# seanwood/gcc-nmf

Hardware: AMD Instinct MI355X
Metric: stereo frames/sec (1024-FFT, K=1024, 100 NMF iters) (higher is better)
Workload: dtype f32; 1 GPU; HBM-resident (float32 samples in HBM -> separated float32 waveforms in HBM; the host-to-host rates are the host_to_host_* fields of a --full run): 64 x 10 s stereo @16 kHz synthetic mixtures per GPU (SURVEY 8d recipe), 1024-pt FFT hop 256 (F=513, T=622/file), K=1024, 100 KL-NMF iters, 128 TDOAs, 3 targets, independent dictionary per file; dictionary_size=1024, parallelism=file-sharded x1, no data-path collective

## Files before the change

### gcc_nmf_amd/csrc/common.h

```cpp
#pragma once
#include <hip/hip_runtime.h>
#include <stdint.h>

#define GCCNMF_OK 0
#define GCCNMF_ERR_ARG 1
#define GCCNMF_ERR_LAUNCH 2
#define GCCNMF_ERR_UNSUPPORTED 3

static inline int gccnmf_ceil_div(int a, int b) { return (a + b - 1) / b; }
static inline int gccnmf_round_up(int a, int b) { return gccnmf_ceil_div(a, b) * b; }

#define GCCNMF_CHECK_LAUNCH()                                   \
    do {                                                        \
        hipError_t e__ = hipGetLastError();                     \
        if (e__ != hipSuccess) return GCCNMF_ERR_LAUNCH;        \
    } while (0)

struct GccNmfPitches {
    int Fp, Kp, Np, Tp;
};

static inline GccNmfPitches gccnmf_make_pitches(int F, int T, int K) {
    GccNmfPitches p;
    p.Fp = gccnmf_round_up(F, 16);
    p.Kp = gccnmf_round_up(K, 64);
    p.Np = gccnmf_round_up(2 * T, 64);
    p.Tp = gccnmf_round_up(T, 64);
    return p;
}

#define GCCNMF_TUNE_KEYS 26
struct GccNmfTune {
    int v[GCCNMF_TUNE_KEYS];
};
extern thread_local GccNmfTune gccnmf_tune;
struct GccNmfCall {
    GccNmfCall();
    ~GccNmfCall();
};
#define GCCNMF_ENTER() GccNmfCall gccnmf_call_scope_
#define gccnmf_tune_ablate (gccnmf_tune.v[1])
#define gccnmf_tune_tile_policy (gccnmf_tune.v[2])
#define gccnmf_tune_dma (gccnmf_tune.v[3])
#define gccnmf_tune_ring (gccnmf_tune.v[4])
#define gccnmf_tune_wh_splits (gccnmf_tune.v[5])
#define gccnmf_tune_rht_splits (gccnmf_tune.v[6])
#define gccnmf_tune_exact_div (gccnmf_tune.v[7])
#define gccnmf_tune_shared_groups (gccnmf_tune.v[8])
#define gccnmf_tune_tail_split (gccnmf_tune.v[9])
#define gccnmf_tune_direct (gccnmf_tune.v[10])
#define gccnmf_tune_direct_tile (gccnmf_tune.v[11])
#define gccnmf_tune_direct_batch (gccnmf_tune.v[12])
#define gccnmf_tune_direct_depth (gccnmf_tune.v[13])
#define gccnmf_tune_short_updh (gccnmf_tune.v[14])
#define gccnmf_tune_fft_r16 (gccnmf_tune.v[15])
#define gccnmf_tune_fused_k12 (gccnmf_tune.v[16])
#define gccnmf_tune_fused_k34 (gccnmf_tune.v[17])
#define gccnmf_tune_persistent (gccnmf_tune.v[18])
#define gccnmf_tune_prefetch (gccnmf_tune.v[19])
#define gccnmf_tune_wide_update_w (gccnmf_tune.v[20])
#define gccnmf_tune_chain (gccnmf_tune.v[21])
#define gccnmf_tune_chain_solo (gccnmf_tune.v[22])
#define gccnmf_tune_chain_rag (gccnmf_tune.v[23])
#define gccnmf_tune_chain_chunk (gccnmf_tune.v[24])
#define gccnmf_tune_chain_fault (gccnmf_tune.v[25])
```

### gcc_nmf_amd/csrc/gemm_dma.h

```cpp
#pragma once
#include <mutex>
#include <type_traits>
#include "gemm_mfma.h"
#include "chain_sync.h"

#ifndef GEMM_DMA_ABL
#define GEMM_DMA_ABL 0
#endif

typedef __attribute__((address_space(3))) void* gemm_lds_ptr;
typedef __attribute__((address_space(1))) const void* gemm_glb_ptr;

__device__ __forceinline__ void gemm_dma16(const float* wave_uniform_base, unsigned lane_byte_offset, unsigned lds_wave_byte_addr) {
    asm volatile("s_mov_b32 m0, %2\n\tglobal_load_lds_dwordx4 %0, %1"
                 :
                 : "v"(lane_byte_offset), "s"(wave_uniform_base), "s"(lds_wave_byte_addr)
                 : "memory");
}

__device__ __forceinline__ void gemm_dma16_masked(const float* wave_uniform_base, unsigned lane_byte_offset, unsigned lds_wave_byte_addr,
                                                  unsigned long long wave_uniform_mask) {
    unsigned long long saved;
    asm volatile("s_mov_b64 %0, exec\n\ts_mov_b64 exec, %4\n\ts_mov_b32 m0, %3\n\tglobal_load_lds_dwordx4 %1, %2\n\ts_mov_b64 exec, %0"
                 : "=&s"(saved)
// ... 86 lines not shown
            if constexpr (NT == 4) v[e][1] = gemm_lds_read2_b32<64, 96>(base + 4 * e * ROWS);
        }
    }
    __device__ __forceinline__ void tie() {
#pragma unroll
        for (int e = 0; e < 4; ++e)
#pragma unroll
            for (int h = 0; h < NT / 2; ++h) gemm_tie(v[e][h]);
    }
    __device__ __forceinline__ void clear() {
#pragma unroll
        for (int e = 0; e < 4; ++e)
#pragma unroll
            for (int h = 0; h < NT / 2; ++h) v[e][h] = gemm_f32x2{0.f, 0.f};
    }
    __device__ __forceinline__ float get(int m, int e) const { return v[e][m >> 1][m & 1]; }
    __device__ __forceinline__ void scale(const gemm_f32x4& s) {
#pragma unroll
        for (int e = 0; e < 4; ++e)
#pragma unroll
            for (int h = 0; h < NT / 2; ++h) v[e][h] *= s[e];
    }
};

__device__ __forceinline__ float gemm_div_fast(float v, float d) {
    const float r = __builtin_amdgcn_rcpf(d);
    const float q = v * r;
    return fmaf(fmaf(-d, q, v), r, q);
}

typedef int gemm_i32x4 __attribute__((ext_vector_type(4)));
__device__ float gemm_buffer_load(gemm_i32x4 rsrc, int voffset, int soffset, int aux) __asm("llvm.amdgcn.raw.buffer.load.f32");
__device__ gemm_f32x4 gemm_buffer_load4(gemm_i32x4 rsrc, int voffset, int soffset, int aux) __asm("llvm.amdgcn.raw.buffer.load.v4f32");
__device__ void gemm_buffer_store(float data, gemm_i32x4 rsrc, int voffset, int soffset, int aux) __asm("llvm.amdgcn.raw.buffer.store.f32");
__device__ __forceinline__ gemm_i32x4 gemm_buffer_rsrc(const void* wave_uniform_base, long bytes = 0x7fffffffL) {
    const unsigned long long a = (unsigned long long)wave_uniform_base;
    gemm_i32x4 r;
    r.x = __builtin_amdgcn_readfirstlane((int)(unsigned)a);
    r.y = __builtin_amdgcn_readfirstlane((int)(unsigned)(a >> 32) & 0xffff);
    r.z = __builtin_amdgcn_readfirstlane((int)(bytes < 0x7fffffffL ? bytes : 0x7fffffffL));
    r.w = 0x00020000;
    return r;
}

template <int EPI, int BM = 512>
struct GemmEpiloguePair {
// ... 236 lines not shown
        q = idx / wt;
        const int w = idx - q * wt;
        tm = w / p.wide_n;
        col0 = (w - tm * p.wide_n) * 64 + 32 * half;
    } else {
        const int r = t - (len + s), base_r = list * p.cr;
        const int lenr = min(max(p.batch * p.rag * p.tiles_m - base_r, 0), p.cr);
        if (r >= lenr) return false;
        const int idx = base_r + r;
        q = idx / p.tiles_m;
        tm = idx - q * p.tiles_m;
        col0 = (p.tiles_n - 1) * 64;
        nw = 1;
    }
    file = gemm_dma_list_file(p, q) + p.file0;
    return true;
}

template <int TM>
struct GemmDmaLds {
    static constexpr int SBUF = 128 * TM * 16 + 64 * 16 + 16 + 16;
};

template <bool A_KC, bool B_KC, int EPI, bool TAIL, int TM, bool NARROW>
__device__ __forceinline__ void gemm_dma_workgroup(const GemmArgs& p, float* const smem, float* const s_rowvec, unsigned* const s_arrivals_p,
                                                   int* const s_ticket, const int list, int t, const GemmSync& sync, const int sync_it = 0,
                                                   const bool trace_on = true) {
    static_assert(TM == 4 || TM == 2, "");
    static_assert(TM == 4 || EPI != EPI_UPDW, "the fused W update owns all rows of its atoms: full-height tiles only");
    static_assert(!NARROW || (EPI != EPI_UPDW && TM == 4), "narrow items: full-height tiles with an element-wise epilogue");
    constexpr int BK = 16, BM = 128 * TM, BN = 64, RW = 32 * TM;
    constexpr int NA = 2 * TM;
    constexpr int SA = BM * BK, SB = BN * BK;
    constexpr int SBUF = SA + SB + BK + BK;
    static_assert(SBUF == GemmDmaLds<TM>::SBUF, "");
    constexpr bool SCALE = !B_KC && (EPI == EPI_DIV || EPI == EPI_STORE);
    unsigned& s_arrivals = *s_arrivals_p;

    int tid = threadIdx.x, lane = tid & 63;
    const int wave = __builtin_amdgcn_readfirstlane(tid >> 6);
    const int wm = wave, wn = 0;
    int l31 = lane & 31, hh = lane >> 5;
#ifdef GCCNMF_EXPERIMENTS
    const bool persistent = p.tickets != nullptr;
#else
    constexpr bool persistent = false;
#endif
// ... 269 lines not shown
        if (TAIL) {
            tail_acc = fmaf(t4.x, tb4.x, tail_acc);
            tail_acc = fmaf(t4.y, tb4.y, tail_acc);
            tail_acc = fmaf(t4.z, tb4.z, tail_acc);
            tail_acc = fmaf(t4.w, tb4.w, tail_acc);
        }
        if (B_KC) rowsum_acc += (rs4.x + rs4.y) + (rs4.z + rs4.w);
        __builtin_amdgcn_sched_barrier(0);
        GEMM_PROBE(6);
        wait_group0();
#ifdef GEMM_DMA_PROBE
        __builtin_amdgcn_sched_barrier(0);
        const unsigned long long pt7 = __builtin_amdgcn_s_memtime();
        probe[0] += pt1 - pt0;
        probe[1] += pt2 - pt1;
        probe[2] += pt3 - pt2;
        probe[3] += pt4 - pt3;
        probe[4] += pt5 - pt4;
        probe[5] += pt6 - pt5;
        probe[6] += pt7 - pt6;
        __builtin_amdgcn_sched_barrier(0);
#endif
    };
    auto main_loop = [&](auto nw_c) {
        for (int kt = 0; kt < nkt; kt += 2) {
            step(std::integral_constant<int, 0>{}, nw_c, kt);
            if (kt + 1 < nkt) step(std::integral_constant<int, 1>{}, nw_c, kt + 1);
        }
    };

    if (SCALE) {
        if (!p.bscale && tid < 2 * BK) smem[(tid >> 4) * SBUF + SA + SB + BK + (tid & 15)] = 1.f;
    }
    bool have = take_item(t);
    if (have) set_offsets(lane);
    bool prefetched = false;
    int it = 0;
    long long* trace_row = nullptr;
    while (have) {
        const int vb = p.lists == 8 ? 8 * t + list : t;
        trace_row = (trace_on && p.trace && vb < p.trace_rows) ? p.trace + 8 * (long)vb : nullptr;
        if (trace_row && tid == 0) {
            trace_row[0] = trace_row[1] = __builtin_amdgcn_s_memrealtime();
            trace_row[4] = (long long)((__builtin_amdgcn_s_getreg((3 << 11) | 20) & 15u) << 16 | (__builtin_amdgcn_s_getreg((31 << 11) | 4) & 0xffffu));
            trace_row[7] = (long long)blockIdx.x << 16 | (long long)it;
        }
#ifdef GCCNMF_EXPERIMENTS
        set_lane_constants(gemm_opaque_tid());
        if (it > 0) set_offsets(lane);
        a0.clear(); a1.clear(); b0.clear(); b1.clear();
        sc0 = sc1 = t4 = tb4 = ts4 = rs4 = zero4;
        tbxy = tbzw = gemm_f32x2{0.f, 0.f};
#else
        set_lane_constants(tid);
#endif
        gemm_sync_wait(sync, file, col0, tid, sync_it, list, n_sync);
        if (trace_row && tid == 0) trace_row[1] = __builtin_amdgcn_s_memrealtime();
        if (!prefetched) {
#pragma unroll
            for (int i = 0; i < NPIECES; ++i) dma_piece(i, 0, 0);
        }
#pragma unroll
        for (int m = 0; m < TM; ++m)
#pragma unroll
            for (int n = 0; n < 2; ++n)
#pragma unroll
                for (int r = 0; r < 16; ++r) acc[m][n][r] = 0.f;
        tail_acc = 0.f;
        rowsum_acc = 0.f;
        if constexpr (EPI == EPI_STORE || EPI == EPI_UPDH) {
#pragma unroll
            for (int i = 0; i < BM / 256; ++i) {
                const int lr = tid + 256 * i, row = min(row0 + lr, p.M - 1);
                s_rowvec[lr] = p.ktailA ? p.ktailA[file * p.s_ktailA + row] : 0.f;
                if (EPI == EPI_UPDH) {
                    const float rd = 1.0f / (p.E2[file * p.sE2 + row] + p.alpha + p.eps);
                    s_rowvec[BM + lr] = p.E1 ? p.E1[file * p.sE1 + row] * rd : rd;
                }
            }
        }
        if (tid == 0) {
            s_arrivals = 0;
            if (persistent) s_ticket[it & 1] = p.wpl + (int)__hip_atomic_fetch_add(p.tickets + list, 1u, __ATOMIC_RELAXED, __HIP_MEMORY_SCOPE_AGENT);
        }
        asm volatile("s_waitcnt vmcnt(0)" ::: "memory");
        __syncthreads();
        read_group0(lds0);
        wait_group0();

        if constexpr (NARROW) {
            if (nw == 1) main_loop(std::integral_constant<int, 1>{});
            else main_loop(std::integral_constant<int, 2>{});
        } else {
            main_loop(std::integral_constant<int, 2>{});
        }
        __syncthreads();
        if (trace_row && tid == 0) trace_row[2] = __builtin_amdgcn_s_memrealtime();

        const int e_file = file, e_row0 = row0, e_col0 = col0, e_nw = nw, e_n = n_item;
        const bool e_active = wave_active, e_tail = do_tail, e_rowsum = do_rowsum;
        have = false;
        prefetched = false;
        if (persistent) {
            t = __builtin_amdgcn_readfirstlane(s_ticket[it & 1]);
            have = take_item(t);
            if (have && p.prefetch) {
                set_offsets(gemm_opaque_tid() & 63);
#pragma unroll
                for (int i = 0; i < NPIECES; ++i) dma_piece(i, 0, 0);
                prefetched = true;
            }
// ... 66 lines not shown
            __syncthreads();
            if (tid == 0) trace_row[3] = __builtin_amdgcn_s_memrealtime();
        }
        gemm_sync_signal(sync, e_file, e_col0, e_nw, tid);
        ++it;
        if (have) __syncthreads();
    }
#ifdef GEMM_DMA_PROBE
    if (p.trace && lane == 0 && (long)p.trace_grid + 4L * blockIdx.x + 4 <= p.trace_rows) {
#pragma unroll
        for (int i = 0; i < 7; ++i) p.trace[8 * ((long)p.trace_grid + blockIdx.x * 4 + wave) + i] = (long long)probe[i];
        p.trace[8 * ((long)p.trace_grid + blockIdx.x * 4 + wave) + 7] = it;
    }
#endif
    if (persistent && tid == 0) {
        const unsigned gone = __hip_atomic_fetch_add(p.tickets + 8, 1u, __ATOMIC_ACQ_REL, __HIP_MEMORY_SCOPE_AGENT);
        if (gone == gridDim.x - 1) {
#pragma unroll
            for (int i = 0; i < 9; ++i) __hip_atomic_store(p.tickets + i, 0u, __ATOMIC_RELAXED, __HIP_MEMORY_SCOPE_AGENT);
        }
    }
}

template <bool A_KC, bool B_KC, int EPI, bool TAIL, int TM, bool NARROW>
__global__ __launch_bounds__(256, 2) void gccnmf_gemm_dma_kernel(GemmArgs p) {
    __shared__ __attribute__((aligned(16))) float smem[2 * GemmDmaLds<TM>::SBUF];
    __shared__ __attribute__((aligned(16))) float s_rowvec[(EPI == EPI_STORE || EPI == EPI_UPDH) ? 2 * 128 * TM : 4];
    __shared__ unsigned s_arrivals;
    __shared__ int s_ticket[2];
    const int list = p.lists == 8 ? (int)(blockIdx.x & 7) : 0;
    const int t = p.lists == 8 ? (int)(blockIdx.x >> 3) : (int)blockIdx.x;
    GemmSync none = {};
    gemm_dma_workgroup<A_KC, B_KC, EPI, TAIL, TM, NARROW>(p, smem, s_rowvec, &s_arrivals, s_ticket, list, t, none);
}

struct GemmChain {
    int first[5];
    int it0, iterations;
    int trace_it;
    GemmSync sync[4];
};
template <bool TAIL, int STAGES, int TM1>
__global__ __launch_bounds__(256, 2) void gccnmf_gemm_chain_kernel(GemmArgs p0, GemmArgs p1, GemmArgs p2, GemmArgs p3, GemmChain ch) {
    static_assert(STAGES == 2 || STAGES == 4, "");
    __shared__ __attribute__((aligned(16))) float smem[2 * GemmDmaLds<4>::SBUF];
    __shared__ __attribute__((aligned(16))) float s_rowvec[2 * 512];
    __shared__ unsigned s_arrivals;
    __shared__ int s_ticket[2];
    const int list = (int)(blockIdx.x & 7);
    int pos = (int)(blockIdx.x >> 3), it = ch.it0;
    if (ch.iterations > 1) {
        const int q = pos / ch.first[4];
        it += q;
        pos -= q * ch.first[4];
    }
    const bool tr = it == ch.trace_it;
    if (pos < ch.first[1]) {
        gemm_dma_workgroup<true, false, EPI_DIV, TAIL, 4, true>(p0, smem, s_rowvec, &s_arrivals, s_ticket, list, pos, ch.sync[0], it, tr);
    } else if (pos < ch.first[2]) {
        gemm_dma_workgroup<false, false, EPI_UPDH, false, TM1, TM1 == 4>(p1, smem, s_rowvec, &s_arrivals, s_ticket, list, pos - ch.first[1], ch.sync[1], it, tr);
    } else if constexpr (STAGES == 4) {
        if (pos < ch.first[3]) {
            gemm_dma_workgroup<true, false, EPI_DIV, TAIL, 4, true>(p2, smem, s_rowvec, &s_arrivals, s_ticket, list, pos - ch.first[2], ch.sync[2], it, tr);
        } else {
            gemm_dma_workgroup<true, true, EPI_UPDW, TAIL, 4, false>(p3, smem, s_rowvec, &s_arrivals, s_ticket, list, pos - ch.first[3], ch.sync[3], it, tr);
        }
    }
}

#ifdef GCCNMF_EXPERIMENTS
unsigned* gccnmf_ticket_block(hipStream_t stream);
#endif

static int gemm_dma_plan(GemmArgs& a, bool narrow_capable, int TM, int whole_files = 0) {
    a.tiles_m = gccnmf_ceil_div(a.M, 128 * TM);
    a.tiles_n = gccnmf_ceil_div(a.N, 64);
    a.lists = (a.xcd_affine && a.batch >= 8) ? 8 : 1;
    const int policy = gccnmf_tune_tail_split;
    const bool narrow_ok = narrow_capable && TM == 4 && policy != 0;
    a.narrow_ok = narrow_ok ? 1 : 0;
    const long tiles = (long)a.batch * a.tiles_m * a.tiles_n;
    if (tiles > (1L << 28)) return -1;
    a.rag = (narrow_ok && a.tiles_n >= 2 && a.N - (a.tiles_n - 1) * 64 <= 32) ? 1 : 0;
    if (a.rag && policy == 1 && !a.concurrent) {
        const long slots = a.lists == 8 ? 64 : 512;
        const long plain = (tiles + a.lists - 1) / a.lists;
        const long with_rag = ((long)a.batch * a.tiles_m * (a.tiles_n - 1) + a.lists - 1) / a.lists + ((long)a.batch * a.tiles_m + a.lists - 1) / a.lists;
        if ((with_rag + slots - 1) / slots > (plain + slots - 1) / slots) a.rag = 0;
// ... 22 lines not shown
    constexpr bool NARROW = false;
#else
    constexpr bool NARROW = TM == 4 && (EPI == EPI_DIV || EPI == EPI_UPDH || EPI == EPI_STORE);
#endif
    const int classic_grid = gemm_dma_plan(a, NARROW, TM);
    if (classic_grid < 1) return GCCNMF_ERR_ARG;
    a.trace = gccnmf_trace_buf;
    a.trace_rows = gccnmf_trace_buf ? gccnmf_trace_blocks : 0;
    a.trace_grid = classic_grid;
    a.tickets = nullptr;
    a.prefetch = 0;
    a.wpl = 0;
    int grid = classic_grid;
#ifdef GCCNMF_EXPERIMENTS
    a.prefetch = gccnmf_tune_prefetch;
    if (gccnmf_tune_persistent && TM == 4 && classic_grid > 512) {
        a.tickets = gccnmf_ticket_block(stream);
        if (a.tickets) {
            grid = 512;
            a.wpl = 512 / a.lists;
        }
    }
#endif
    hipLaunchKernelGGL((gccnmf_gemm_dma_kernel<A_KC, B_KC, EPI, TAIL, TM, NARROW>), dim3(grid), dim3(256), 0, stream, a);
    GCCNMF_CHECK_LAUNCH();
    return GCCNMF_OK;
}

template <bool A_KC, bool B_KC, int EPI, bool TAIL>
static int gccnmf_launch_gemm_dma(GemmArgs a, hipStream_t stream) {
    if (!a.A || !a.B || !a.C || a.M < 1 || a.N < 1 || a.Kd < 1 || a.batch < 1) return GCCNMF_ERR_ARG;
    if ((a.lda & 3) || (a.ldb & 3)) return GCCNMF_ERR_ARG;
    a.ablate = gccnmf_tune_ablate;
    a.exact_div = gccnmf_tune_exact_div;
    if constexpr (EPI != EPI_UPDW) {
        if ((a.M <= 256 && gccnmf_tune_tail_split != 0) || gccnmf_tune_tail_split == 3) return gccnmf_launch_gemm_dma_tm<A_KC, B_KC, EPI, TAIL, 2>(a, stream);
        const long tpf = (long)gccnmf_ceil_div(a.M, 512) * gccnmf_ceil_div(a.N, 64);
        const long total = tpf * a.batch, rounds = total / 512;
        if (gccnmf_tune_tail_split == 1 && !gccnmf_trace_buf && !a.concurrent && a.M > 256) {
            auto full_cost = [](long tiles) { const long r = tiles % 512; return (tiles / 512) * 250 + (r == 0 ? 0 : r <= 256 ? 135 : 250); };
            auto half_cost = [](long halves) {
                const long r = halves % 768;
                return (halves / 768) * 190 + (r == 0 ? 0 : r <= 256 ? 85 : r <= 512 ? 135 : 190);
            };
            const long plain = full_cost(total), all_half = half_cost(2 * total);
            long split = 1L << 40;
            const int head = (int)(rounds * 512 / tpf);
// ... 17 lines not shown
```

### gcc_nmf_amd/csrc/gemm_mfma.h

```cpp
#pragma once
#include "common.h"

typedef float f32x16 __attribute__((ext_vector_type(16)));

#ifndef GEMM_VARIANT
#define GEMM_VARIANT 2
#endif
#if GEMM_VARIANT & 1
#define GEMM_PRIO(x) __builtin_amdgcn_s_setprio(x)
#else
#define GEMM_PRIO(x)
#endif
#if GEMM_VARIANT & 2
#define GEMM_PIN()
#else
#define GEMM_PIN() __builtin_amdgcn_sched_barrier(0)
#endif

extern long long* gccnmf_trace_buf;
extern int gccnmf_trace_blocks;

enum GemmEpilogue {
    EPI_STORE = 0,
    EPI_DIV = 1,
// ... 34 lines not shown
    const float* E0;
    long sE0;
    const float* E1;
    long sE1;
    const float* E2;
    long sE2;
    const float2* X;
    long sX;
    float alpha, eps;
    int T, Tp, Fp, ldv;
    long long* trace;
    int lists;
    int cw, cr;
    int split;
    int rag, wide_n;
    int whole_files;
    const int* ragged_n;
    const int* ragged_lists;
    int ragged_kd;
    int narrow_ok;
    int wpl, prefetch;
    unsigned* tickets;
    int trace_rows, trace_grid;
};

template <int EPI>
__device__ __forceinline__ bool gemm_col_valid(const GemmArgs& p, int col) {
    if (EPI == EPI_PHASE) {
        int ic = col / p.Tp;
        return col < p.N && (col - ic * p.Tp) < p.T;
    }
    return col < p.N;
}

template <int EPI>
__device__ __forceinline__ void gemm_epilogue(const GemmArgs& p, int file, int row, int col, float acc) {
    if (EPI == EPI_STORE) {
        p.C[file * p.sC + (long)row * p.ldc + col] = acc;
    } else if (EPI == EPI_DIV) {
        long idx = (long)row * p.ldc + col;
        p.C[file * p.sC + idx] = p.E0[file * p.sE0 + idx] / acc;
    } else if (EPI == EPI_UPDH) {
        long idx = file * p.sC + (long)row * p.ldc + col;
        float h = p.C[idx];
        if (p.E1) h *= p.E1[file * p.sE1 + row];
        float den = p.E2[file * p.sE2 + row] + p.alpha + p.eps;
// ... 543 lines not shown
```

### gcc_nmf_amd/csrc/nmf.hip

```cpp
#include <mutex>
#include "gemm_ring.h"
#include "direct.h"
#include "update_w.h"
#ifdef GCCNMF_EXPERIMENTS
int gccnmf_launch_gemm_stream(GemmArgs a, hipStream_t stream);
#endif
int gccnmf_klnmf_fixed_launch(const float* V, const float* W, float* H, float* workspace, int F, int N, int K, int batch, int iterations,
                              float alpha, float eps, bool ones, hipStream_t s);
bool gccnmf_klnmf_fixed_supported(int F, int K);
long gccnmf_klnmf_fixed_workspace_floats(int F, int K);
#include "../../include/gccnmf_hip.h"

#include <atomic>
#include <algorithm>
#include <vector>
#define GCCNMF_SHARED_STREAMS 4
#define GCCNMF_CHAIN_MAX_ITERATIONS gccnmf_tune_chain_chunk
#define GCCNMF_RAGGED_MAX_BATCH 248
#define GCCNMF_SPLITS 4
#define GCCNMF_DIRECT_MAX_BATCH 8
struct GccNmfKnob {
    int def, lo, hi, experiment;
};
static const GccNmfKnob gccnmf_knobs[GCCNMF_TUNE_KEYS] = {
// ... 3 lines not shown
    {1, 0, 1, 0},
    {1, 0, 1, 1},
    {3, 1, 4, 1},
    {4, 1, 4, 1},
    {1, 0, 1, 0},
    {3, 1, GCCNMF_SHARED_STREAMS, 0},
    {1, 0, 3, 0},
    {1, 0, 1, 0},
    {0, 0, 8, 1},
    {4, 1, GCCNMF_DIRECT_MAX_BATCH, 0},
    {0, 0, 4, 1},
    {1, 0, 1, 1},
    {1, 0, 1, 1},
    {1, 0, 2, 0},
    {1, 0, 2, 0},
    {0, 0, 1, 1},
    {1, 0, 1, 1},
    {1, 0, 1, 1},
    {1, 0, 8, 0},
    {0, 0, 1, 1},
    {1, 0, 3, 0},
    {2048, 1, 65536, 0},
    {0, 0, 1, 1},
};
static std::atomic<int> gccnmf_knob_value[GCCNMF_TUNE_KEYS];
static std::atomic<int> gccnmf_knobs_ready{0};
static void gccnmf_knobs_init() {
    static std::mutex mu;
    if (gccnmf_knobs_ready.load(std::memory_order_acquire)) return;
    std::lock_guard<std::mutex> lock(mu);
    if (gccnmf_knobs_ready.load(std::memory_order_relaxed)) return;
    for (int k = 0; k < GCCNMF_TUNE_KEYS; ++k) gccnmf_knob_value[k].store(gccnmf_knobs[k].def, std::memory_order_relaxed);
    gccnmf_knobs_ready.store(1, std::memory_order_release);
}
static GccNmfTune gccnmf_tune_load() {
    gccnmf_knobs_init();
    GccNmfTune t;
    for (int k = 0; k < GCCNMF_TUNE_KEYS; ++k) t.v[k] = gccnmf_knob_value[k].load(std::memory_order_relaxed);
    return t;
}
thread_local GccNmfTune gccnmf_tune = gccnmf_tune_load();
static thread_local int gccnmf_call_depth = 0;
GccNmfCall::GccNmfCall() {
    if (gccnmf_call_depth++ == 0) gccnmf_tune = gccnmf_tune_load();
}
GccNmfCall::~GccNmfCall() { --gccnmf_call_depth; }
// ... 291 lines not shown
struct NmfGeom {
    int F, N, K, Fp, Kp, Np;
    int ld;
    int Fm;
    bool tail;
    long sV, sW, sH, sU;
};

static NmfGeom make_geom(int F, int N, int K) {
    NmfGeom g;
    GccNmfPitches p = gccnmf_make_pitches(F, 1, K);
    g.F = F; g.N = N; g.K = K;
    g.Fp = p.Fp; g.Kp = p.Kp; g.Np = gccnmf_round_up(N, 64);
    g.ld = g.Np;
    g.tail = (F % 128) == 1 && F > 1;
    g.Fm = g.tail ? F - 1 : F;
    g.sV = (long)g.Fp * g.Np;
    g.sW = (long)g.Fp * g.Kp;
    g.sH = (long)g.Kp * g.Np;
    g.sU = (long)g.Fp * g.Kp;
    return g;
}

static int launch_wh_div(const NmfGeom& g, const float* V, const float* W, long sW, const float* H, const float* hscale,
                         long sScale, float* R, int batch, int xcd, hipStream_t s) {
    GemmArgs a = {};
    a.A = W; a.sA = sW; a.lda = g.Kp; a.a_clamp = g.Fp - 1;
    a.B = H; a.sB = g.sH; a.ldb = g.ld; a.b_clamp = g.Np - 4;
    a.M = g.Fm; a.N = g.N; a.Kd = g.K;
    a.batch = batch; a.xcd_affine = xcd & 1; a.concurrent = (xcd >> 1) & 1;
    a.bscale = hscale; a.s_bscale = sScale;
    a.tail_row = g.F - 1;
    a.C = R; a.sC = g.sV; a.ldc = g.ld;
    a.E0 = V; a.sE0 = g.sV;
    return dispatch_gemm<true, false, EPI_DIV>(a, g.tail, s);
}

static int launch_update_h(const NmfGeom& g, const float* W, long sW, const float* R, float* H, const float* hscale,
                           long sScale, const float* colsumW, long sVec, float alpha, float eps, int batch, int xcd,
                           hipStream_t s) {
    GemmArgs a = {};
    a.A = W; a.sA = sW; a.lda = g.Kp; a.a_clamp = g.Kp - 4;
    a.B = R; a.sB = g.sV; a.ldb = g.ld; a.b_clamp = g.Np - 4;
    a.M = g.K; a.N = g.N; a.Kd = g.F;
    if ((g.F % 16) == 1) {
        a.Kd = g.F - 1;
        a.ktailA = W + (long)(g.F - 1) * g.Kp; a.s_ktailA = sW;
        a.ktailB = R + (long)(g.F - 1) * g.ld; a.s_ktailB = g.sV;
    }
    a.batch = batch; a.xcd_affine = xcd & 1; a.concurrent = (xcd >> 1) & 1;
    a.C = H; a.sC = g.sH; a.ldc = g.ld;
    a.E1 = hscale; a.sE1 = sScale;
    a.E2 = colsumW; a.sE2 = sVec;
    a.alpha = alpha; a.eps = eps;
    return dispatch_gemm<false, false, EPI_UPDH>(a, false, s);
}

static int launch_rht(const NmfGeom& g, const float* R, const float* H, float* U, float* rowsumH, int batch, int xcd,
                      hipStream_t s) {
    GemmArgs a = {};
    a.A = R; a.sA = g.sV; a.lda = g.ld; a.a_clamp = g.Fp - 1;
    a.B = H; a.sB = g.sH; a.ldb = g.ld; a.b_clamp = g.Kp - 1;
    a.M = g.Fm; a.N = g.K; a.Kd = g.N;
    a.batch = batch; a.xcd_affine = xcd & 1; a.concurrent = (xcd >> 1) & 1;
    a.tail_row = g.F - 1;
    a.rowsumB = rowsumH; a.s_rowsumB = g.Kp;
    a.C = U; a.sC = g.sU; a.ldc = g.Kp;
    return dispatch_gemm<true, true, EPI_STORE>(a, g.tail, s);
}

static bool can_fuse_w_update(const NmfGeom& g, int batch) {
    if (g.Fm <= 128 || g.Fm > 512 || gccnmf_tune_tile_policy == 2) return false;
    return gccnmf_tune_tile_policy == 1 || (long)batch * gccnmf_ceil_div(g.K, 64) >= 256;
}

static int launch_rht_update_w(const NmfGeom& g, const float* R, const float* H, float* W, float* colsumW, float* hscale, int batch,
                               int xcd, hipStream_t s) {
    GemmArgs a = {};
    a.A = R; a.sA = g.sV; a.lda = g.ld; a.a_clamp = g.Fp - 1;
    a.B = H; a.sB = g.sH; a.ldb = g.ld; a.b_clamp = g.Kp - 1;
    a.M = g.Fm; a.N = g.K; a.Kd = g.N;
    a.batch = batch; a.xcd_affine = xcd & 1; a.concurrent = (xcd >> 1) & 1;
    a.tail_row = g.F - 1;
    a.C = W; a.sC = g.sW; a.ldc = g.Kp;
    a.out_colsum = colsumW; a.out_norm = hscale; a.s_out = g.Kp;
    if (gccnmf_tune_dma && (a.M & 127) == 0 && (a.N & 63) == 0)
        return g.tail ? gccnmf_launch_gemm_dma<true, true, EPI_UPDW, true>(a, s) : gccnmf_launch_gemm_dma<true, true, EPI_UPDW, false>(a, s);
    return g.tail ? gccnmf_launch_gemm<4, 1, true, true, EPI_UPDW, true>(a, s) : gccnmf_launch_gemm<4, 1, true, true, EPI_UPDW, false>(a, s);
}

#ifdef GCCNMF_EXPERIMENTS

__global__ __launch_bounds__(256) void nmf_div_partials_kernel(const float* __restrict__ V, const float* __restrict__ P, long sP,
                                                               int nsplit, int F, int N, int Np, float* __restrict__ R) {
    const int n4 = Np / 4;
    const long idx = (long)blockIdx.x * 256 + threadIdx.x;
    if (idx >= (long)F * n4) return;
    const int f = (int)(idx / n4), n = 4 * (int)(idx - (long)f * n4);
    if (n >= N) return;
    const long i = (long)f * Np + n;
    float4 d = *(const float4*)(P + i);
// ... 218 lines not shown
    return any_size || can_fuse_w_update(g, batch);
}
static bool chain_rule(int batch, int flags) {
    if (flags & 4) return false;
    const int longest = (batch + 7) / 8;
    return batch >= 24 && 100L * 8 * longest <= 108L * batch;
}

struct RaggedPlan {
    const int* n;
    int lists[8][GEMM_RAGGED_LMAX + 1];
    const int* d_n;
    const int* d_lists;
};

static int launch_klnmf_chain(int stages, const NmfGeom& g, const float* V, float* W, float* H, float* R, float* colsumW, float* hscale,
                              float alpha, float eps, int batch, int flags, unsigned* counters, int it0, int iterations, hipStream_t s,
                              const RaggedPlan* rg = nullptr) {
    GemmArgs a[4] = {};
    const int concurrent = (flags & 4) ? 1 : 0;
    for (int i = 0; i < 4; ++i) {
        a[i].batch = batch; a[i].xcd_affine = 1; a[i].concurrent = concurrent;
        a[i].ablate = gccnmf_tune_ablate; a[i].exact_div = gccnmf_tune_exact_div;
    }
    for (int i = 0; i < 3; i += 2) {
        a[i].A = W; a[i].sA = g.sW; a[i].lda = g.Kp; a[i].a_clamp = g.Fp - 1;
        a[i].B = H; a[i].sB = g.sH; a[i].ldb = g.ld; a[i].b_clamp = g.Np - 4;
        a[i].M = g.Fm; a[i].N = g.N; a[i].Kd = g.K;
        a[i].tail_row = g.F - 1;
        a[i].C = R; a[i].sC = g.sV; a[i].ldc = g.ld;
        a[i].E0 = V; a[i].sE0 = g.sV;
    }
    a[0].bscale = hscale; a[0].s_bscale = g.Kp;
    a[1].A = W; a[1].sA = g.sW; a[1].lda = g.Kp; a[1].a_clamp = g.Kp - 4;
    a[1].B = R; a[1].sB = g.sV; a[1].ldb = g.ld; a[1].b_clamp = g.Np - 4;
    a[1].M = g.K; a[1].N = g.N; a[1].Kd = g.F - 1;
    a[1].ktailA = W + (long)(g.F - 1) * g.Kp; a[1].s_ktailA = g.sW;
    a[1].ktailB = R + (long)(g.F - 1) * g.ld; a[1].s_ktailB = g.sV;
    a[1].C = H; a[1].sC = g.sH; a[1].ldc = g.ld;
    a[1].E1 = hscale; a[1].sE1 = g.Kp;
    a[1].E2 = colsumW; a[1].sE2 = g.Kp;
    a[1].alpha = alpha; a[1].eps = eps;
    a[3].A = R; a[3].sA = g.sV; a[3].lda = g.ld; a[3].a_clamp = g.Fp - 1;
    a[3].B = H; a[3].sB = g.sH; a[3].ldb = g.ld; a[3].b_clamp = g.Kp - 1;
    a[3].M = g.Fm; a[3].N = g.K; a[3].Kd = g.N;
    a[3].tail_row = g.F - 1;
// ... 48 lines not shown
        ch.sync[2].sig_cnt = c34; ch.sync[2].sig_stride = 1; ch.sync[2].sig_per_tile = 0;
        ch.sync[3].wait_cnt = c34; ch.sync[3].wait_stride = 1; ch.sync[3].wait_per_tile = 0;
        ch.sync[3].wait_need = (unsigned)(a[2].tiles_m * (rg ? 1 : a[2].tiles_n));
        ch.sync[3].wait_scale_tiles = rg ? 1 : 0;
        {
            ch.sync[3].sig_cnt = c41; ch.sync[3].sig_stride = 1; ch.sync[3].sig_per_tile = 0;
            ch.sync[0].wait_cnt = c41; ch.sync[0].wait_stride = 1; ch.sync[0].wait_per_tile = 0; ch.sync[0].wait_lag = 1;
            ch.sync[0].wait_need = (unsigned)(a[3].tiles_m * a[3].tiles_n);
        }
    }
    if (iterations > 1 && stages != 4) return GCCNMF_ERR_ARG;
    if (it0 == 0 && iterations == 1) ch.sync[0].wait_cnt = nullptr;
    ch.it0 = it0; ch.iterations = iterations;
    ch.trace_it = it0 + (iterations > 4 ? iterations - 3 : iterations - 1);
    if ((long)8 * ch.first[4] * iterations > (1L << 30)) return GCCNMF_ERR_ARG;
    for (int i = 0; i < stages; ++i) {
        a[i].trace = gccnmf_trace_buf ? gccnmf_trace_buf + 8L * 8 * ch.first[i] : nullptr;
        a[i].trace_rows = gccnmf_trace_buf ? gccnmf_trace_blocks - 8 * ch.first[i] : 0;
        if (a[i].trace_rows <= 0) a[i].trace = nullptr;
    }
    const int grid = 8 * ch.first[4] * iterations;
    const unsigned pad = gccnmf_tune_chain_solo ? 16384u : 0u;
    if (!g.tail) return GCCNMF_ERR_ARG;
    if (stages == 2 && tm1 == 4) hipLaunchKernelGGL((gccnmf_gemm_chain_kernel<true, 2, 4>), dim3(grid), dim3(256), pad, s, a[0], a[1], a[2], a[3], ch);
    else if (stages == 2) hipLaunchKernelGGL((gccnmf_gemm_chain_kernel<true, 2, 2>), dim3(grid), dim3(256), pad, s, a[0], a[1], a[2], a[3], ch);
    else if (tm1 == 4) hipLaunchKernelGGL((gccnmf_gemm_chain_kernel<true, 4, 4>), dim3(grid), dim3(256), pad, s, a[0], a[1], a[2], a[3], ch);
    else hipLaunchKernelGGL((gccnmf_gemm_chain_kernel<true, 4, 2>), dim3(grid), dim3(256), pad, s, a[0], a[1], a[2], a[3], ch);
    GCCNMF_CHECK_LAUNCH();
    return GCCNMF_OK;
}

static int short_chain_group(const NmfGeom& g, int batch, int flags) {
    const int want = gccnmf_tune_chain;
    if (!want || want == 2 || want == 4 || !gccnmf_tune_fused_k12 || !gccnmf_tune_fused_k34 || gccnmf_tune_tile_policy != 0) return 0;
    if (direct_path(g, batch) || (flags & 3) || batch < 8 || !g.tail || g.Fm < 64 || g.Fm > 512 || (g.Fm % 64) != 0 || g.K > 128) return 0;
    if ((g.Fm / 64) * 16 < 32 * gccnmf_ceil_div(g.K, 32) || g.F > 64 * 9 || !gccnmf_tune_ring || (long)batch * (g.Kp / 64) >= 256) return 0;
    if (want == 1 && !(chain_rule(batch, flags) && fused_wh_updh(g, batch, flags) && fused_whdiv_rht_files(g, batch, flags) == batch)) return 0;
    if (gccnmf_tune_ablate == 64) return 0;
    return ((long)batch * (g.Kp / 32) >= 256 && gccnmf_tune_wide_update_w) ? 32 : 16;
}

static int launch_short_chain(const NmfGeom& g, const float* V, float* W, float* H, float* U, float* colsumW, float* rowsumH, float* hscale,
                              float alpha, float eps, int batch, int group, unsigned* counters, int it0, int iterations, hipStream_t s) {
    ShortChainArgs c = {};
    c.a12.W = W; c.a12.sW = g.sW; c.a12.lda = g.Kp;
    c.a12.H = H; c.a12.sH = g.sH; c.a12.ldb = g.ld;
    c.a12.V = V; c.a12.sV = g.sV; c.a12.ldv = g.ld;
    c.a12.scale = hscale; c.a12.colsum = colsumW; c.a12.sVec = g.Kp;
    c.a12.M = g.Fm; c.a12.N = g.N; c.a12.Kd = g.K; c.a12.batch = batch;
    c.a12.alpha = alpha; c.a12.eps = eps;
// ... 674 lines not shown
```

Measured before the change: 155,400 frames/s.

## Emulate fp32 GEMMs with split-bf16 MFMA (six-term bf16x3 product)

Adds a bf16 path to the DMA GEMM workgroup. Each fp32 operand fragment is split into hi/mid/lo bf16 pieces, and the product is accumulated with six 32x32x16 bf16 MFMAs per tile step instead of fp32 MFMAs. The DMA, barrier and LDS reads are rescheduled into fixed slots across the MFMA sequence. A new tune knob turns the path on for K>=256, covering both the standalone and chained kernels. The aim is to use the much higher bf16 matrix throughput. The cost is extra VALU work for the splits, more registers, and a small loss of accuracy versus true fp32.

```diff
diff --git a/gcc_nmf_amd/csrc/common.h b/gcc_nmf_amd/csrc/common.h
--- a/gcc_nmf_amd/csrc/common.h
+++ b/gcc_nmf_amd/csrc/common.h
@@ -29,7 +29,7 @@
     return p;
 }
 
-#define GCCNMF_TUNE_KEYS 26
+#define GCCNMF_TUNE_KEYS 27
 struct GccNmfTune {
     int v[GCCNMF_TUNE_KEYS];
 };
@@ -64,3 +64,4 @@
 #define gccnmf_tune_chain_rag (gccnmf_tune.v[23])
 #define gccnmf_tune_chain_chunk (gccnmf_tune.v[24])
 #define gccnmf_tune_chain_fault (gccnmf_tune.v[25])
+#define gccnmf_tune_split_bf16 (gccnmf_tune.v[26])
diff --git a/gcc_nmf_amd/csrc/gemm_dma.h b/gcc_nmf_amd/csrc/gemm_dma.h
--- a/gcc_nmf_amd/csrc/gemm_dma.h
+++ b/gcc_nmf_amd/csrc/gemm_dma.h
@@ -132,6 +132,38 @@
             for (int h = 0; h < NT / 2; ++h) v[e][h] *= s[e];
     }
 };
+
+typedef __bf16 gemm_bf16x2 __attribute__((ext_vector_type(2)));
+typedef __bf16 gemm_bf16x8 __attribute__((ext_vector_type(8)));
+typedef unsigned gemm_u32x4 __attribute__((ext_vector_type(4)));
+struct GemmSplit8 {
+    gemm_u32x4 hi, mid, lo;
+};
+__device__ __forceinline__ void gemm_split2(gemm_f32x2 x, unsigned& hi, unsigned& mid, unsigned& lo) {
+    const gemm_bf16x2 h = __builtin_convertvector(x, gemm_bf16x2);
+    const gemm_f32x2 r = x - __builtin_convertvector(h, gemm_f32x2);
+    const gemm_bf16x2 m = __builtin_convertvector(r, gemm_bf16x2);
+    const gemm_f32x2 r2 = r - __builtin_convertvector(m, gemm_f32x2);
+    const gemm_bf16x2 l = __builtin_convertvector(r2, gemm_bf16x2);
+    hi = __builtin_bit_cast(unsigned, h);
+    mid = __builtin_bit_cast(unsigned, m);
+    lo = __builtin_bit_cast(unsigned, l);
+}
+__device__ __forceinline__ GemmSplit8 gemm_split8(const float (&x)[8]) {
+    GemmSplit8 s;
+#pragma unroll
+    for (int i = 0; i < 4; ++i) {
+        unsigned h, m, l;
+        gemm_split2(gemm_f32x2{x[2 * i], x[2 * i + 1]}, h, m, l);
+        s.hi[i] = h;
+        s.mid[i] = m;
+        s.lo[i] = l;
+    }
+    return s;
+}
+__host__ __device__ constexpr int gemm_bf16x6_a(int term) { return term == 0 ? 2 : (term == 2 || term == 3) ? 1 : 0; }
+__host__ __device__ constexpr int gemm_bf16x6_b(int term) { return term == 1 ? 2 : (term == 2 || term == 4) ? 1 : 0; }
+__device__ __forceinline__ const gemm_u32x4& gemm_bf16x6_piece(const GemmSplit8& s, int which) { return which == 0 ? s.hi : which == 1 ? s.mid : s.lo; }
 
 __device__ __forceinline__ float gemm_div_fast(float v, float d) {
     const float r = __builtin_amdgcn_rcpf(d);
@@ -414,7 +446,7 @@
     static constexpr int SBUF = 128 * TM * 16 + 64 * 16 + 16 + 16;
 };
 
-template <bool A_KC, bool B_KC, int EPI, bool TAIL, int TM, bool NARROW>
+template <bool A_KC, bool B_KC, int EPI, bool TAIL, int TM, bool NARROW, bool BF16>
 __device__ __forceinline__ void gemm_dma_workgroup(const GemmArgs& p, float* const smem, float* const s_rowvec, unsigned* const s_arrivals_p,
                                                    int* const s_ticket, const int list, int t, const GemmSync& sync, const int sync_it = 0,
                                                    const bool trace_on = true) {
@@ -730,10 +762,179 @@
         __builtin_amdgcn_sched_barrier(0);
 #endif
     };
+    constexpr int BF_SLOTS = 6 * TM;
+    constexpr int BF_DMA_SLOTS = (NPIECES + 1) / 2;
+    constexpr int BF_READ = TM == 4 ? 7 : 0;
+    constexpr int BF_ARR = TM == 4 ? 12 : 6;
+    constexpr int BF_WAIT = TM == 4 ? 18 : 9;
+    static_assert(BF_DMA_SLOTS + 2 <= BF_ARR && BF_ARR < BF_WAIT - 1 && BF_WAIT <= BF_SLOTS - 3, "");
+    GemmFrag<A_KC, 2, BM> ah0g0, ah0g1, ah1g0, ah1g1;
+    constexpr unsigned HALF1 = A_KC ? 2 * 2048 : 4 * 64;
+    auto bf_read_b = [&](const unsigned lds) {
+        if (wave_active) {
+            b0.read(lds + oB0);
+            b1.read(lds + oB1);
+        }
+        if (SCALE) {
+            sc0 = gemm_lds_read_b128<4 * (SA + SB + BK)>(lds + 16 * hh);
+            sc1 = gemm_lds_read_b128<4 * (SA + SB + BK) + 32>(lds + 16 * hh);
+        }
+    };
+    auto bf_wait_b = [&]() {
+        gemm_wait_lds();
+        b0.tie();
+        b1.tie();
+        if (SCALE) {
+            gemm_tie(sc0);
+            gemm_tie(sc1);
+            b0.scale(sc0);
+            b1.scale(sc1);
+        }
+    };
+    auto bf_read_side = [&](const unsigned lds) {
+        if (TAIL) {
+            t4 = gemm_lds_read_b128<4 * (SA + SB)>(lds + 16 * tg);
+            if (B_KC) {
+                tb4 = gemm_lds_read_b128<0>(lds + oTB);
+            } else {
+                tbxy = gemm_lds_read2_b32<0 * BN, 1 * BN>(lds + oTB);
+                tbzw = gemm_lds_read2_b32<2 * BN, 3 * BN>(lds + oTB);
+                if (SCALE) ts4 = gemm_lds_read_b128<4 * (SA + SB + BK)>(lds + 16 * tg);
+            }
+        }
+        if (B_KC) rs4 = gemm_lds_read_b128<0>(lds + oRS);
+    };
+    auto bf_side = [&]() {
+        if (TAIL) {
+            gemm_tie(t4);
+            if (B_KC) {
+                gemm_tie(tb4);
+            } else {
+                gemm_tie(tbxy);
+                gemm_tie(tbzw);
+                tb4 = gemm_f32x4{tbxy.x, tbxy.y, tbzw.x, tbzw.y};
+                if (SCALE) {
+                    gemm_tie(ts4);
+                    tb4 *= ts4;
+                }
+            }
+            tail_acc = fmaf(t4.x, tb4.x, tail_acc);
+            tail_acc = fmaf(t4.y, tb4.y, tail_acc);
+            tail_acc = fmaf(t4.z, tb4.z, tail_acc);
+            tail_acc = fmaf(t4.w, tb4.w, tail_acc);
+        }
+        if (B_KC) {
+            gemm_tie(rs4);
+            rowsum_acc += (rs4.x + rs4.y) + (rs4.z + rs4.w);
+        }
+    };
+    auto bf_read_a = [&](const unsigned lds, auto half_c) {
+        if (wave_active) {
+            if constexpr (decltype(half_c)::value == 0) {
+                ah0g0.read(lds + oA0);
+                ah0g1.read(lds + oA1);
+            } else {
+                ah1g0.read(lds + oA0 + HALF1);
+                ah1g1.read(lds + oA1 + HALF1);
+            }
+        }
+    };
+    auto bf_tie_a = [&](auto half_c) {
+        if constexpr (decltype(half_c)::value == 0) {
+            ah0g0.tie();
+            ah0g1.tie();
+        } else {
+            ah1g0.tie();
+            ah1g1.tie();
+        }
+    };
+    auto step_bf16 = [&](auto cur_c, auto nw_c, const int kt) {
+        constexpr int CUR = decltype(cur_c)::value;
+        constexpr int NW = decltype(nw_c)::value;
+        const unsigned ldsC = lds0 + 4 * CUR * SBUF, ldsN = lds0 + 4 * (CUR ^ 1) * SBUF;
+        const int ktn = min(kt + 1, nkt - 1);
+        GemmSplit8 bs[2], as;
+        if (wave_active) {
+#pragma unroll
+            for (int n = 0; n < NW; ++n) {
+                float x[8];
+#pragma unroll
+                for (int e = 0; e < 4; ++e) {
+                    x[e] = b0.get(n, e);
+                    x[4 + e] = b1.get(n, e);
+                }
+                bs[n] = gemm_split8(x);
+            }
+        }
+        __builtin_amdgcn_sched_barrier(0);
+        unsigned seen = 0;
+#pragma unroll
+        for (int slot = 0; slot < BF_SLOTS; ++slot) {
+            const int m = slot / 6, term = slot % 6;
+            if (slot < BF_DMA_SLOTS) {
+                dma_piece(2 * slot, ktn, CUR ^ 1);
+                if (2 * slot + 1 < NPIECES) dma_piece(2 * slot + 1, ktn, CUR ^ 1);
+                __builtin_amdgcn_sched_barrier(0);
+            }
+            if (slot == BF_ARR) {
+                __builtin_amdgcn_sched_barrier(0);
+                gemm_wait_lds();
+                if constexpr (TM == 4) bf_tie_a(std::integral_constant<int, 1>{});
+                bf_side();
+                asm volatile("s_waitcnt vmcnt(0)" ::: "memory");
+                gemm_barrier_arrive(arrivals_addr);
+                __builtin_amdgcn_sched_barrier(0);
+            }
+            if (slot == BF_WAIT - 1) {
+                __builtin_amdgcn_sched_barrier(0);
+                seen = gemm_barrier_peek(arrivals_addr);
+                __builtin_amdgcn_sched_barrier(0);
+            }
+            if (slot == BF_READ) {
+                __builtin_amdgcn_sched_barrier(0);
+                if constexpr (TM == 4) bf_read_a(ldsC, std::integral_constant<int, 1>{});
+                bf_read_side(ldsC);
+                __builtin_amdgcn_sched_barrier(0);
+            }
+            if (wave_active && term == 0) {
+                const GemmFrag<A_KC, 2, BM>& g0 = m < 2 ? ah0g0 : ah1g0;
+                const GemmFrag<A_KC, 2, BM>& g1 = m < 2 ? ah0g1 : ah1g1;
+                float x[8];
+#pragma unroll
+                for (int e = 0; e < 4; ++e) {
+                    x[e] = g0.get(m & 1, e);
+                    x[4 + e] = g1.get(m & 1, e);
+                }
+                as = gemm_split8(x);
+            }
+            if (slot == BF_WAIT) {
+                __builtin_amdgcn_sched_barrier(0);
+                gemm_barrier_wait(arrivals_addr, 4u * (unsigned)(kt + 1), seen);
+                bf_read_b(ldsN);
+                bf_read_a(ldsN, std::integral_constant<int, 0>{});
+                __builtin_amdgcn_sched_barrier(0);
+            }
+            if (wave_active) {
+#pragma unroll
+                for (int n = 0; n < NW; ++n)
+                    acc[m][n] = __builtin_amdgcn_mfma_f32_32x32x16_bf16(__builtin_bit_cast(gemm_bf16x8, gemm_bf16x6_piece(as, gemm_bf16x6_a(term))),
+                                                                        __builtin_bit_cast(gemm_bf16x8, gemm_bf16x6_piece(bs[n], gemm_bf16x6_b(term))),
+                                                                        acc[m][n], 0, 0, 0);
+            }
+        }
+        __builtin_amdgcn_sched_barrier(0);
+        bf_wait_b();
+        bf_tie_a(std::integral_constant<int, 0>{});
+    };
     auto main_loop = [&](auto nw_c) {
         for (int kt = 0; kt < nkt; kt += 2) {
-            step(std::integral_constant<int, 0>{}, nw_c, kt);
-            if (kt + 1 < nkt) step(std::integral_constant<int, 1>{}, nw_c, kt + 1);
+            if constexpr (BF16) {
+                step_bf16(std::integral_constant<int, 0>{}, nw_c, kt);
+                if (kt + 1 < nkt) step_bf16(std::integral_constant<int, 1>{}, nw_c, kt + 1);
+            } else {
+                step(std::integral_constant<int, 0>{}, nw_c, kt);
+                if (kt + 1 < nkt) step(std::integral_constant<int, 1>{}, nw_c, kt + 1);
+            }
         }
     };
 
@@ -757,6 +958,7 @@
         set_lane_constants(gemm_opaque_tid());
         if (it > 0) set_offsets(lane);
         a0.clear(); a1.clear(); b0.clear(); b1.clear();
+        if constexpr (BF16) { ah0g0.clear(); ah0g1.clear(); ah1g0.clear(); ah1g1.clear(); }
         sc0 = sc1 = t4 = tb4 = ts4 = rs4 = zero4;
         tbxy = tbzw = gemm_f32x2{0.f, 0.f};
 #else
@@ -793,8 +995,15 @@
         }
         asm volatile("s_waitcnt vmcnt(0)" ::: "memory");
         __syncthreads();
-        read_group0(lds0);
-        wait_group0();
+        if constexpr (BF16) {
+            bf_read_b(lds0);
+            bf_read_a(lds0, std::integral_constant<int, 0>{});
+            bf_wait_b();
+            bf_tie_a(std::integral_constant<int, 0>{});
+        } else {
+            read_group0(lds0);
+            wait_group0();
+        }
 
         if constexpr (NARROW) {
             if (nw == 1) main_loop(std::integral_constant<int, 1>{});
@@ -907,7 +1116,7 @@
     }
 }
 
-template <bool A_KC, bool B_KC, int EPI, bool TAIL, int TM, bool NARROW>
+template <bool A_KC, bool B_KC, int EPI, bool TAIL, int TM, bool NARROW, bool BF16>
 __global__ __launch_bounds__(256, 2) void gccnmf_gemm_dma_kernel(GemmArgs p) {
     __shared__ __attribute__((aligned(16))) float smem[2 * GemmDmaLds<TM>::SBUF];
     __shared__ __attribute__((aligned(16))) float s_rowvec[(EPI == EPI_STORE || EPI == EPI_UPDH) ? 2 * 128 * TM : 4];
@@ -916,7 +1125,7 @@
     const int list = p.lists == 8 ? (int)(blockIdx.x & 7) : 0;
     const int t = p.lists == 8 ? (int)(blockIdx.x >> 3) : (int)blockIdx.x;
     GemmSync none = {};
-    gemm_dma_workgroup<A_KC, B_KC, EPI, TAIL, TM, NARROW>(p, smem, s_rowvec, &s_arrivals, s_ticket, list, t, none);
+    gemm_dma_workgroup<A_KC, B_KC, EPI, TAIL, TM, NARROW, BF16>(p, smem, s_rowvec, &s_arrivals, s_ticket, list, t, none);
 }
 
 struct GemmChain {
@@ -925,7 +1134,7 @@
     int trace_it;
     GemmSync sync[4];
 };
-template <bool TAIL, int STAGES, int TM1>
+template <bool TAIL, int STAGES, int TM1, bool BF16>
 __global__ __launch_bounds__(256, 2) void gccnmf_gemm_chain_kernel(GemmArgs p0, GemmArgs p1, GemmArgs p2, GemmArgs p3, GemmChain ch) {
     static_assert(STAGES == 2 || STAGES == 4, "");
     __shared__ __attribute__((aligned(16))) float smem[2 * GemmDmaLds<4>::SBUF];
@@ -941,14 +1150,14 @@
     }
     const bool tr = it == ch.trace_it;
     if (pos < ch.first[1]) {
-        gemm_dma_workgroup<true, false, EPI_DIV, TAIL, 4, true>(p0, smem, s_rowvec, &s_arrivals, s_ticket, list, pos, ch.sync[0], it, tr);
+        gemm_dma_workgroup<true, false, EPI_DIV, TAIL, 4, true, BF16>(p0, smem, s_rowvec, &s_arrivals, s_ticket, list, pos, ch.sync[0], it, tr);
     } else if (pos < ch.first[2]) {
-        gemm_dma_workgroup<false, false, EPI_UPDH, false, TM1, TM1 == 4>(p1, smem, s_rowvec, &s_arrivals, s_ticket, list, pos - ch.first[1], ch.sync[1], it, tr);
+        gemm_dma_workgroup<false, false, EPI_UPDH, false, TM1, TM1 == 4, BF16>(p1, smem, s_rowvec, &s_arrivals, s_ticket, list, pos - ch.first[1], ch.sync[1], it, tr);
     } else if constexpr (STAGES == 4) {
         if (pos < ch.first[3]) {
-            gemm_dma_workgroup<true, false, EPI_DIV, TAIL, 4, true>(p2, smem, s_rowvec, &s_arrivals, s_ticket, list, pos - ch.first[2], ch.sync[2], it, tr);
+            gemm_dma_workgroup<true, false, EPI_DIV, TAIL, 4, true, BF16>(p2, smem, s_rowvec, &s_arrivals, s_ticket, list, pos - ch.first[2], ch.sync[2], it, tr);
         } else {
-            gemm_dma_workgroup<true, true, EPI_UPDW, TAIL, 4, false>(p3, smem, s_rowvec, &s_arrivals, s_ticket, list, pos - ch.first[3], ch.sync[3], it, tr);
+            gemm_dma_workgroup<true, true, EPI_UPDW, TAIL, 4, false, BF16>(p3, smem, s_rowvec, &s_arrivals, s_ticket, list, pos - ch.first[3], ch.sync[3], it, tr);
         }
     }
 }
@@ -1017,7 +1226,8 @@
         }
     }
 #endif
-    hipLaunchKernelGGL((gccnmf_gemm_dma_kernel<A_KC, B_KC, EPI, TAIL, TM, NARROW>), dim3(grid), dim3(256), 0, stream, a);
+    if (a.split_bf16) hipLaunchKernelGGL((gccnmf_gemm_dma_kernel<A_KC, B_KC, EPI, TAIL, TM, NARROW, true>), dim3(grid), dim3(256), 0, stream, a);
+    else hipLaunchKernelGGL((gccnmf_gemm_dma_kernel<A_KC, B_KC, EPI, TAIL, TM, NARROW, false>), dim3(grid), dim3(256), 0, stream, a);
     GCCNMF_CHECK_LAUNCH();
     return GCCNMF_OK;
 }
diff --git a/gcc_nmf_amd/csrc/gemm_mfma.h b/gcc_nmf_amd/csrc/gemm_mfma.h
--- a/gcc_nmf_amd/csrc/gemm_mfma.h
+++ b/gcc_nmf_amd/csrc/gemm_mfma.h
@@ -80,6 +80,7 @@
     int wpl, prefetch;
     unsigned* tickets;
     int trace_rows, trace_grid;
+    int split_bf16;
 };
 
 template <int EPI>
diff --git a/gcc_nmf_amd/csrc/nmf.hip b/gcc_nmf_amd/csrc/nmf.hip
--- a/gcc_nmf_amd/csrc/nmf.hip
+++ b/gcc_nmf_amd/csrc/nmf.hip
@@ -49,6 +49,7 @@
     {1, 0, 3, 0},
     {2048, 1, 65536, 0},
     {0, 0, 1, 1},
+    {1, 0, 2, 0},
 };
 static std::atomic<int> gccnmf_knob_value[GCCNMF_TUNE_KEYS];
 static std::atomic<int> gccnmf_knobs_ready{0};
@@ -386,9 +387,12 @@
     return g;
 }
 
+static int split_bf16_for(const NmfGeom& g) { return gccnmf_tune_split_bf16 == 2 || (gccnmf_tune_split_bf16 == 1 && g.K >= 256) ? 1 : 0; }
+
 static int launch_wh_div(const NmfGeom& g, const float* V, const float* W, long sW, const float* H, const float* hscale,
                          long sScale, float* R, int batch, int xcd, hipStream_t s) {
     GemmArgs a = {};
+    a.split_bf16 = split_bf16_for(g);
     a.A = W; a.sA = sW; a.lda = g.Kp; a.a_clamp = g.Fp - 1;
     a.B = H; a.sB = g.sH; a.ldb = g.ld; a.b_clamp = g.Np - 4;
     a.M = g.Fm; a.N = g.N; a.Kd = g.K;
@@ -404,6 +408,7 @@
                            long sScale, const float* colsumW, long sVec, float alpha, float eps, int batch, int xcd,
                            hipStream_t s) {
     GemmArgs a = {};
+    a.split_bf16 = split_bf16_for(g);
     a.A = W; a.sA = sW; a.lda = g.Kp; a.a_clamp = g.Kp - 4;
     a.B = R; a.sB = g.sV; a.ldb = g.ld; a.b_clamp = g.Np - 4;
     a.M = g.K; a.N = g.N; a.Kd = g.F;
@@ -423,6 +428,7 @@
 static int launch_rht(const NmfGeom& g, const float* R, const float* H, float* U, float* rowsumH, int batch, int xcd,
                       hipStream_t s) {
     GemmArgs a = {};
+    a.split_bf16 = split_bf16_for(g);
     a.A = R; a.sA = g.sV; a.lda = g.ld; a.a_clamp = g.Fp - 1;
     a.B = H; a.sB = g.sH; a.ldb = g.ld; a.b_clamp = g.Kp - 1;
     a.M = g.Fm; a.N = g.K; a.Kd = g.N;
@@ -441,6 +447,7 @@
 static int launch_rht_update_w(const NmfGeom& g, const float* R, const float* H, float* W, float* colsumW, float* hscale, int batch,
                                int xcd, hipStream_t s) {
     GemmArgs a = {};
+    a.split_bf16 = split_bf16_for(g);
     a.A = R; a.sA = g.sV; a.lda = g.ld; a.a_clamp = g.Fp - 1;
     a.B = H; a.sB = g.sH; a.ldb = g.ld; a.b_clamp = g.Kp - 1;
     a.M = g.Fm; a.N = g.K; a.Kd = g.N;
@@ -705,6 +712,7 @@
     for (int i = 0; i < 4; ++i) {
         a[i].batch = batch; a[i].xcd_affine = 1; a[i].concurrent = concurrent;
         a[i].ablate = gccnmf_tune_ablate; a[i].exact_div = gccnmf_tune_exact_div;
+        a[i].split_bf16 = split_bf16_for(g);
     }
     for (int i = 0; i < 3; i += 2) {
         a[i].A = W; a[i].sA = g.sW; a[i].lda = g.Kp; a[i].a_clamp = g.Fp - 1;
@@ -799,10 +807,18 @@
     const int grid = 8 * ch.first[4] * iterations;
     const unsigned pad = gccnmf_tune_chain_solo ? 16384u : 0u;
     if (!g.tail) return GCCNMF_ERR_ARG;
-    if (stages == 2 && tm1 == 4) hipLaunchKernelGGL((gccnmf_gemm_chain_kernel<true, 2, 4>), dim3(grid), dim3(256), pad, s, a[0], a[1], a[2], a[3], ch);
-    else if (stages == 2) hipLaunchKernelGGL((gccnmf_gemm_chain_kernel<true, 2, 2>), dim3(grid), dim3(256), pad, s, a[0], a[1], a[2], a[3], ch);
-    else if (tm1 == 4) hipLaunchKernelGGL((gccnmf_gemm_chain_kernel<true, 4, 4>), dim3(grid), dim3(256), pad, s, a[0], a[1], a[2], a[3], ch);
-    else hipLaunchKernelGGL((gccnmf_gemm_chain_kernel<true, 4, 2>), dim3(grid), dim3(256), pad, s, a[0], a[1], a[2], a[3], ch);
+    auto launch = [&](auto kernel) { hipLaunchKernelGGL(kernel, dim3(grid), dim3(256), pad, s, a[0], a[1], a[2], a[3], ch); };
+    if (a[0].split_bf16) {
+        if (stages == 2 && tm1 == 4) launch(gccnmf_gemm_chain_kernel<true, 2, 4, true>);
+        else if (stages == 2) launch(gccnmf_gemm_chain_kernel<true, 2, 2, true>);
+        else if (tm1 == 4) launch(gccnmf_gemm_chain_kernel<true, 4, 4, true>);
+        else launch(gccnmf_gemm_chain_kernel<true, 4, 2, true>);
+    } else {
+        if (stages == 2 && tm1 == 4) launch(gccnmf_gemm_chain_kernel<true, 2, 4, false>);
+        else if (stages == 2) launch(gccnmf_gemm_chain_kernel<true, 2, 2, false>);
+        else if (tm1 == 4) launch(gccnmf_gemm_chain_kernel<true, 4, 4, false>);
+        else launch(gccnmf_gemm_chain_kernel<true, 4, 2, false>);
+    }
     GCCNMF_CHECK_LAUNCH();
     return GCCNMF_OK;
 }
```

New measurement: 61520 frames/s, median of 2. 0.396x the previous value.
